# Jianxff/svo_pro_universal

Measured on AMD Instinct MI355X. Metric: aligned patches/sec + ms/frame, EuRoC 640x480 mono, 1/2/4/8 MI355X, higher is better.
Workload: dtype f64

## Files before the change

### svo_pro_universal_amd/csrc/context.hip

```cpp
#include <cmath>
#include <cstdarg>
#include <algorithm>
#include <cstring>

#include "svoh_internal.h"
#include "svoh_math.h"

namespace svoh {

static thread_local std::string g_global_err = "no error";

int set_error(svoh_ctx* ctx, int code, const char* fmt, ...)
{
  char buf[1024];
  va_list ap;
  va_start(ap, fmt);
  vsnprintf(buf, sizeof buf, fmt, ap);
  va_end(ap);
  if (ctx) ctx->err = buf; else g_global_err = buf;
  return code;
}

void set_global_error(const char* msg) { g_global_err = msg; }

// ... 335 lines not shown

__global__ __launch_bounds__(64) void camera_maths_kernel(const svoh_camera cam, int n, const double* xyz, double* px, double* J, double* f_back)
{
  const int i = blockIdx.x * 64 + threadIdx.x;
  if (i >= n) return;
  const CamModel cm = load_camera(cam);
  const Vec3 p = { xyz[3 * i], xyz[3 * i + 1], xyz[3 * i + 2] };
  double u, v;
  project3(cm, p, u, v);
  px[2 * i] = u; px[2 * i + 1] = v;
  double Jl[6];
  project3_jacobian(cm, p, Jl);
  for (int k = 0; k < 6; ++k) J[6 * i + k] = Jl[k];
  const Vec3 f = back_project3(cm, u, v);
  f_back[3 * i] = f.x; f_back[3 * i + 1] = f.y; f_back[3 * i + 2] = f.z;
}

__global__ __launch_bounds__(64) void camera_maths_wide_kernel(const svoh_camera cam, int n, const double* xyz, double* px, double* J, double* f_back)
{
  const int i = blockIdx.x * 64 + threadIdx.x;
  if (i >= n) return;
  const CamModelWide cm = load_camera_wide(cam);
  const Vec3 p = { xyz[3 * i], xyz[3 * i + 1], xyz[3 * i + 2] };
  double u, v;
  project3(cm, p, u, v);
  px[2 * i] = u; px[2 * i + 1] = v;
  if (J) {
    double Jl[6];
    project3_jacobian(cm, p, Jl);
    for (int k = 0; k < 6; ++k) J[6 * i + k] = Jl[k];
  }
  const Vec3 f = back_project3(cm, u, v);
  f_back[3 * i] = f.x; f_back[3 * i + 1] = f.y; f_back[3 * i + 2] = f.z;
}

void load_knobs_from_env(SvohKnobs& k)
{
  auto get = [](const char* name) { const char* e = getenv(name); return e ? atoi(e) : kKnobUnset; };
  k.klt_block = get("SVOH_KLT_BLOCK");
  k.matcher_g8 = get("SVOH_MATCHER_G8");
  k.seed_binning = get("SVOH_SEED_BINNING");
  k.pose_threads = get("SVOH_POSE_THREADS");
  k.align_cluster = get("SVOH_ALIGN_CLUSTER");
#ifdef SVOH_TEST_HOOKS
  k.align_cluster_test_absent = get("SVOH_ALIGN_CLUSTER_TEST_ABSENT");
#endif
  k.align_threads = get("SVOH_ALIGN_THREADS");
  k.align_rows = get("SVOH_ALIGN_ROWS");
  k.align_latency_build = get("SVOH_ALIGN_LATENCY_BUILD");
  k.align_lds = get("SVOH_ALIGN_LDS");
  k.align_wg_per_cu = get("SVOH_ALIGN_WG_PER_CU");
  k.kernel_timing = get("SVOH_KERNEL_TIMING");
  k.copy_kernel = get("SVOH_COPY_KERNEL");
}

static int build_pyramid_levels(svoh_ctx* ctx, hipStream_t stream, const std::shared_ptr<Slab>& slab, uint8_t* base, size_t fbytes, const size_t* offs, const int* ws,
                                const int* hs, int n_images, int width, int height, int n_levels, int rounding, svoh_frame_t* out_frames);

extern "C" {

int svoh_abi_version(void) { return SVOH_ABI_VERSION; }

int svoh_set_kernel_timing(svoh_ctx* ctx, int enabled)
try {
  if (!ctx) return set_error(nullptr, SVOH_ERR_INVALID_ARGUMENT, "ctx is NULL");
  ctx->knobs.kernel_timing = enabled ? 1 : 0;
  return SVOH_OK;
} SVOH_ABI_CATCH(ctx)

int svoh_set_copy_policy(svoh_ctx* ctx, int policy)
try {
  if (!ctx) return set_error(nullptr, SVOH_ERR_INVALID_ARGUMENT, "ctx is NULL");
  SVOH_REQUIRE(ctx, policy >= 0 && policy <= 2, "copy policy: 0 the runtime's copies, 1 copy kernels for 16 KB .. 1 MB, 2 copy kernels always");
  ctx->knobs.copy_kernel = policy;
  return SVOH_OK;
} SVOH_ABI_CATCH(ctx)

int svoh_reload_knobs(svoh_ctx* ctx)
try {
  if (!ctx) return set_error(nullptr, SVOH_ERR_INVALID_ARGUMENT, "ctx is NULL");
  const int timing = ctx->knobs.kernel_timing, copy_policy = ctx->knobs.copy_kernel;
  load_knobs_from_env(ctx->knobs);
  if (ctx->knobs.kernel_timing == kKnobUnset) ctx->knobs.kernel_timing = timing;
  if (ctx->knobs.copy_kernel == kKnobUnset) ctx->knobs.copy_kernel = copy_policy;
  return SVOH_OK;
} SVOH_ABI_CATCH(ctx)

int svoh_create(int device, svoh_ctx** out_ctx)
try {
  if (!out_ctx) return set_error(nullptr, SVOH_ERR_INVALID_ARGUMENT, "out_ctx is NULL");
  *out_ctx = nullptr;
  int n = 0;
  hipError_t e = hipGetDeviceCount(&n);
  if (e != hipSuccess || n <= 0)
    return set_error(nullptr, SVOH_ERR_NO_DEVICE, "no HIP device available (%s); libsvo_hip has no CPU path",
                     e == hipSuccess ? "device count is 0" : hipGetErrorString(e));
  if (device < 0 || device >= n)
    return set_error(nullptr, SVOH_ERR_INVALID_ARGUMENT, "device %d out of range [0,%d)", device, n);
  svoh_ctx* ctx = new (std::nothrow) svoh_ctx();
  if (!ctx) return set_error(nullptr, SVOH_ERR_OUT_OF_MEMORY, "out of host memory");
  ctx->device = device;
  ctx->err = "no error";
  load_knobs_from_env(ctx->knobs);
  e = hipSetDevice(device);
  if (e == hipSuccess) e = hipStreamCreateWithFlags(&ctx->stream, hipStreamNonBlocking);
  for (int k = 0; k < svoh_ctx::kAlignEventRing; ++k) {
    if (e == hipSuccess) e = hipEventCreate(&ctx->ev_align_start[k]);
    if (e == hipSuccess) e = hipEventCreate(&ctx->ev_align_stop[k]);
  }
  if (e == hipSuccess) e = hipEventCreateWithFlags(&ctx->ev_align_staged, hipEventDisableTiming);
  if (e == hipSuccess) e = hipEventCreate(&ctx->ev_misc_start);
  if (e == hipSuccess) e = hipEventCreate(&ctx->ev_misc_stop);
  hipDeviceProp_t prop;
  if (e == hipSuccess) e = hipGetDeviceProperties(&prop, device);
  if (e != hipSuccess) {
    set_error(nullptr, SVOH_ERR_HIP, "context creation failed: %s", hipGetErrorString(e));
    delete ctx;
    return SVOH_ERR_HIP;
  }
  ctx->num_cus = prop.multiProcessorCount;
  ctx->lds_per_block = prop.sharedMemPerBlock;
  *out_ctx = ctx;
  return SVOH_OK;
} SVOH_ABI_CATCH(nullptr)

int svoh_destroy(svoh_ctx* ctx)
try {
  if (!ctx) return SVOH_OK;
  (void)hipSetDevice(ctx->device);
  if (ctx->stream) { (void)hipStreamSynchronize(ctx->stream); }
  if (ctx->upload_stream) { (void)hipStreamSynchronize(ctx->upload_stream); }
  ctx->frames.clear();
  for (auto& kv : ctx->masks) (void)hipFree(kv.second.ptr);
  ctx->masks.clear();
  for (int k = 0; k < svoh_ctx::kAlignEventRing; ++k) {
    if (ctx->ev_align_start[k]) (void)hipEventDestroy(ctx->ev_align_start[k]);
    if (ctx->ev_align_stop[k]) (void)hipEventDestroy(ctx->ev_align_stop[k]);
  }
  if (ctx->ev_align_staged) (void)hipEventDestroy(ctx->ev_align_staged);
  if (ctx->ev_misc_start) (void)hipEventDestroy(ctx->ev_misc_start);
  if (ctx->ev_misc_stop) (void)hipEventDestroy(ctx->ev_misc_stop);
  if (ctx->ev_pose_done) (void)hipEventDestroy(ctx->ev_pose_done);
  if (ctx->ev_features) (void)hipEventDestroy(ctx->ev_features);
  if (ctx->ev_points) (void)hipEventDestroy(ctx->ev_points);
  if (ctx->ev_detect) (void)hipEventDestroy(ctx->ev_detect);
  if (ctx->ev_matcher_done) (void)hipEventDestroy(ctx->ev_matcher_done);
  if (ctx->upload_stream) { (void)hipStreamSynchronize(ctx->upload_stream); (void)hipStreamDestroy(ctx->upload_stream); }
  if (ctx->ev_upload) (void)hipEventDestroy(ctx->ev_upload);
  if (ctx->stream) (void)hipStreamDestroy(ctx->stream);
  delete ctx;
  return SVOH_OK;
} SVOH_ABI_CATCH(ctx)

const char* svoh_last_error_string(const svoh_ctx* ctx)
{
  return ctx ? ctx->err.c_str() : g_global_err.c_str();
}

int svoh_synchronize(svoh_ctx* ctx)
try {
  if (!ctx) return set_error(nullptr, SVOH_ERR_INVALID_ARGUMENT, "ctx is NULL");
  SVOH_HIP_TRY(ctx, hipStreamSynchronize(ctx->stream));
  return SVOH_OK;
} SVOH_ABI_CATCH(ctx)

void* svoh_stream(svoh_ctx* ctx) { return ctx ? (void*)ctx->stream : nullptr; }

int svoh_last_kernel_counters(svoh_ctx* ctx, uint64_t out[8])
try {
  if (!ctx) return set_error(nullptr, SVOH_ERR_INVALID_ARGUMENT, "ctx is NULL");
  SVOH_REQUIRE(ctx, out != nullptr && ctx->misc_launched && ctx->d_counters.ptr, "no counters yet");
  if (ctx->unit_counts_pending) {
    const int rc = reduce_unit_counts_now(ctx, ctx->unit_counts_pending);
    if (rc != SVOH_OK) return rc;
    ctx->unit_counts_pending = 0;
  }
  SVOH_HIP_TRY(ctx, hipMemcpyAsync(out, ctx->d_counters.ptr, 8 * sizeof(uint64_t), hipMemcpyDeviceToHost, ctx->stream));
  SVOH_HIP_TRY(ctx, hipStreamSynchronize(ctx->stream));
  return SVOH_OK;
} SVOH_ABI_CATCH(ctx)

int svoh_last_kernel_ms(svoh_ctx* ctx, float* ms)
try {
  if (!ctx) return set_error(nullptr, SVOH_ERR_INVALID_ARGUMENT, "ctx is NULL");
// ... 262 lines not shown
                                    rounding, out_frame);
  if (rc != SVOH_OK) return rc;
  if (host_levels_out) {
    const Frame* f = find_frame(ctx, *out_frame);
    for (int l = 0; l < n_levels; ++l) {
      if (!host_levels_out[l]) continue;
      SVOH_HIP_TRY(ctx, hipMemcpyAsync(host_levels_out[l], f->lv[l].data, (size_t)f->lv[l].w * f->lv[l].h,
                                       hipMemcpyDeviceToHost, ctx->stream));
    }
    SVOH_HIP_TRY(ctx, hipStreamSynchronize(ctx->stream));
  }
  return SVOH_OK;
} SVOH_ABI_CATCH(ctx)

int svoh_download_level(svoh_ctx* ctx, svoh_frame_t frame, int level, uint8_t* out, int* out_width, int* out_height)
try {
  if (!ctx) return set_error(nullptr, SVOH_ERR_INVALID_ARGUMENT, "ctx is NULL");
  const Frame* f = find_frame(ctx, frame);
  if (!f) return set_error(ctx, SVOH_ERR_BAD_HANDLE, "unknown frame handle %llu", (unsigned long long)frame);
  SVOH_REQUIRE(ctx, level >= 0 && level < f->n_levels, "level out of range");
  if (out_width) *out_width = f->lv[level].w;
  if (out_height) *out_height = f->lv[level].h;
  if (out) {
    SVOH_HIP_TRY(ctx, hipSetDevice(ctx->device));
    SVOH_HIP_TRY(ctx, hipMemcpyAsync(out, f->lv[level].data, (size_t)f->lv[level].w * f->lv[level].h,
                                     hipMemcpyDeviceToHost, ctx->stream));
    SVOH_HIP_TRY(ctx, hipStreamSynchronize(ctx->stream));
  }
  return SVOH_OK;
} SVOH_ABI_CATCH(ctx)

int svoh_frame_info(svoh_ctx* ctx, svoh_frame_t frame, int* n_levels, int* width0, int* height0)
try {
  if (!ctx) return set_error(nullptr, SVOH_ERR_INVALID_ARGUMENT, "ctx is NULL");
  const Frame* f = find_frame(ctx, frame);
  if (!f) return set_error(ctx, SVOH_ERR_BAD_HANDLE, "unknown frame handle %llu", (unsigned long long)frame);
  if (n_levels) *n_levels = f->n_levels;
  if (width0) *width0 = f->lv[0].w;
  if (height0) *height0 = f->lv[0].h;
  return SVOH_OK;
} SVOH_ABI_CATCH(ctx)

int svoh_context_stats(svoh_ctx* ctx, svoh_context_stats_t* out)
try {
  if (!ctx) return set_error(nullptr, SVOH_ERR_INVALID_ARGUMENT, "ctx is NULL");
  SVOH_REQUIRE(ctx, out != nullptr, "NULL argument");
  out->live_frames = (int64_t)ctx->frames.size();
  std::unordered_map<const void*, size_t> slabs;
  for (const auto& kv : ctx->frames)
    if (kv.second.slab) slabs[kv.second.slab.get()] = kv.second.slab->bytes;
  size_t fb = 0;
  for (const auto& kv : slabs) fb += kv.second;
  out->frame_bytes = (int64_t)fb;
  const svoh::DevBuffer* bufs[] = { &ctx->d_desc, &ctx->d_results, &ctx->d_feat, &ctx->d_eval, &ctx->d_xchg, &ctx->d_split,
                                    &ctx->d_counters, &ctx->d_unit_counts, &ctx->d_scratch0, &ctx->d_scratch1, &ctx->d_scratch2, &ctx->d_seed_bin, &ctx->d_match_seeds, &ctx->d_match_direct, &ctx->d_cand, &ctx->d_cand_multi };
  size_t wb = 0;
  for (const svoh::DevBuffer* b : bufs) wb += b->cap;
  out->workspace_bytes = (int64_t)wb;
  return SVOH_OK;
} SVOH_ABI_CATCH(ctx)

int svoh_camera_maths(svoh_ctx* ctx, const svoh_camera* cam, int n, const double* xyz, double* px, double* J, double* f_back)
try {
  if (!ctx) return set_error(nullptr, SVOH_ERR_INVALID_ARGUMENT, "ctx is NULL");
  SVOH_REQUIRE(ctx, cam && xyz && px && n >= 1 && n <= (1 << 20), "bad arguments");
  SVOH_REQUIRE(ctx, camera_is_known(*cam), "unsupported distortion model");
  SVOH_REQUIRE(ctx, cam->distortion != SVOH_DISTORTION_ATAN || (cam->d[0] != 0.0 && std::isfinite(cam->d[0])),
               "ATAN (fisheye) camera: s = d[0] must be finite and non-zero");
  if (J && !camera_has_jacobian(*cam))
    return set_error(ctx, SVOH_ERR_UNSUPPORTED, "the ATAN (fisheye) camera has no Jacobian (AtanDistortion::jacobian): pass J = NULL");
  SVOH_HIP_TRY(ctx, hipSetDevice(ctx->device));
  const size_t nd = (size_t)n;
  SVOH_HIP_TRY(ctx, ctx->d_scratch2.reserve(14 * nd * sizeof(double)));
  double* d = static_cast<double*>(ctx->d_scratch2.ptr);
  SVOH_HIP_TRY(ctx, hipMemcpyAsync(d, xyz, 3 * nd * sizeof(double), hipMemcpyHostToDevice, ctx->stream));
  if (camera_is_narrow(*cam))
    hipLaunchKernelGGL(camera_maths_kernel, dim3((unsigned)((n + 63) / 64)), dim3(64), 0, ctx->stream, *cam, n, d, d + 3 * nd, d + 5 * nd,
                       d + 11 * nd);
  else
    hipLaunchKernelGGL(camera_maths_wide_kernel, dim3((unsigned)((n + 63) / 64)), dim3(64), 0, ctx->stream, *cam, n, d, d + 3 * nd,
                       J ? d + 5 * nd : nullptr, d + 11 * nd);
  const hipError_t e = hipGetLastError();
  if (e != hipSuccess) return set_error(ctx, SVOH_ERR_HIP, "camera_maths launch failed: %s", hipGetErrorString(e));
  SVOH_HIP_TRY(ctx, hipMemcpyAsync(px, d + 3 * nd, 2 * nd * sizeof(double), hipMemcpyDeviceToHost, ctx->stream));
  if (J) SVOH_HIP_TRY(ctx, hipMemcpyAsync(J, d + 5 * nd, 6 * nd * sizeof(double), hipMemcpyDeviceToHost, ctx->stream));
  if (f_back) SVOH_HIP_TRY(ctx, hipMemcpyAsync(f_back, d + 11 * nd, 3 * nd * sizeof(double), hipMemcpyDeviceToHost, ctx->stream));
  SVOH_HIP_TRY(ctx, hipStreamSynchronize(ctx->stream));
  return SVOH_OK;
} SVOH_ABI_CATCH(ctx)

int svoh_release_frame(svoh_ctx* ctx, svoh_frame_t frame)
try {
  if (!ctx) return set_error(nullptr, SVOH_ERR_INVALID_ARGUMENT, "ctx is NULL");
  auto it = ctx->frames.find(frame);
  if (it == ctx->frames.end())
    return set_error(ctx, SVOH_ERR_BAD_HANDLE, "unknown frame handle %llu", (unsigned long long)frame);
  ctx->frames.erase(it);
  ++ctx->handle_generation;
  return SVOH_OK;
} SVOH_ABI_CATCH(ctx)


int svoh_mask_upload(svoh_ctx* ctx, int width, int height, int pitch, const uint8_t* data, svoh_mask_t* out_mask)
try {
  if (!ctx) return set_error(nullptr, SVOH_ERR_INVALID_ARGUMENT, "ctx is NULL");
  SVOH_REQUIRE(ctx, data && out_mask, "NULL argument");
  *out_mask = 0;
// ... 32 lines not shown
```

### svo_pro_universal_amd/csrc/sparse_align.hip

```cpp
#include <atomic>
#include <cstdlib>
#include <cstring>

#include <type_traits>

#include "svoh_internal.h"
#include "svoh_device_utils.h"
#include "svoh_math.h"

#define SVOH_ALIGN_DRAIN(ctx) do { SVOH_HIP_TRY(ctx, hipStreamSynchronize((ctx)->stream)); (ctx)->align_launches_since_drain = 0; } while (0)

namespace svoh {

struct DevCamDesc {
  DevImage ref[SVOH_MAX_LEVELS];
  DevImage cur[SVOH_MAX_LEVELS];
  svoh_camera cam;
  svoh_se3 ref_T_imu_cam, ref_T_cam_imu, cur_T_cam_imu;
  double ref_pos[3];
  const double* px;
  const double* f;
  const double* pos_world;
  const uint8_t* flags;
  int32_t n_features;
  int32_t feat_off;
};

struct DevProblemDesc {
  int32_t n_cams, cam_begin;
  svoh_se3 T_init;
  double alpha_init, beta_init;
  svoh_align_prior prior;
};

struct AlignKernelArgs {
  const DevProblemDesc* problems;
  const DevCamDesc* cams;
  svoh_align_result* results;
  double* wpk;
  int64_t slots;
  uint8_t* wsel;
  uint8_t* wvis;
  svoh_align_options opt;
  int32_t lds_img_bytes;
  int32_t rig_build;
  int32_t latency_build;
  int32_t lds_two_per_cu;
  int32_t ws_lds_bytes;
  int32_t eval_level;
  double* eval_out;
  long long* stamps;
  int32_t n_problems;
  int32_t* queue;
  int32_t one_each;
  const svoh_align_gn_state* ext_state;
  int32_t raw_sums;
  int32_t cluster;
  double* xchg;
  unsigned int* bar;
#ifdef SVOH_TEST_HOOKS
  int32_t cluster_test_absent;
#endif
};

constexpr int kXchgStride = 64;
// ... 1761 lines not shown
  if (!forced && !split && eval_level < 0 && n_problems == 1 && shared_class_geometry(ctx, problems[0], &shared_single)) forced = &shared_single;

  int S = (split && !split->update && split->n_shares > 1) ? split->n_shares : 1;
  bool cluster = false;
  if (!split && eval_level < 0) {
    const int g = forced ? forced->cluster_g : decide_cluster(ctx, n_problems, problems);
    if (g >= 2) { S = g; cluster = true; }
  }
  SVOH_REQUIRE(ctx, !forced || (!split && eval_level < 0), "a forced geometry applies to full runs only");
  SVOH_REQUIRE(ctx, !cluster || (int64_t)S * n_problems <= ctx->num_cus, "cluster mode: more workgroups than compute units");
  SVOH_REQUIRE(ctx, !cluster || n_problems <= kClusterMaxProblems, "cluster mode: more problems in one launch than arrival counters");
  SVOH_REQUIRE(ctx, S == 1 || n_problems == 1 || cluster, "shares apply to a single problem");
  const int n_desc = n_problems * S;

  size_t n_cams_total = 0, n_feat_total = 0, host_bytes = 0;
  int n_pos_jobs = 0;
  LaunchShape shape;
  for (int p = 0; p < n_problems; ++p) {
    const svoh_align_problem& pb = problems[p];
    SVOH_REQUIRE(ctx, pb.n_cams >= 1 && pb.n_cams <= SVOH_MAX_CAMS, "n_cams out of range");
    int nf = 0;
    for (int c = 0; c < pb.n_cams; ++c) {
      const svoh_align_camera& cam = pb.cams[c];
      SVOH_REQUIRE(ctx, cam.n_features >= 0, "negative n_features");
      SVOH_REQUIRE(ctx, cam.n_features == 0 || (cam.px && cam.f && cam.pos_world && cam.flags),
                   "NULL feature array");
      SVOH_REQUIRE(ctx, cam.cam.distortion == SVOH_DISTORTION_NONE || cam.cam.distortion == SVOH_DISTORTION_RADTAN,
                   "unsupported distortion model");
      nf += cam.n_features;
      if (cam.mem_space == SVOH_MEM_HOST && !(split && split->update))
        host_bytes += ((size_t)cam.n_features * (8 * 8 + 1) + 63) & ~(size_t)63;
      if (cam.pos_seed_unit) {
        SVOH_REQUIRE(ctx, cam.mem_space == SVOH_MEM_HOST && !split && eval_level < 0, "pos_seed_unit: host-memory cameras of full runs only");
        host_bytes += (((size_t)cam.n_features * 4 + 63) & ~(size_t)63) + 64;
        ++n_pos_jobs;
      }
    }
    n_cams_total += (size_t)pb.n_cams * S;
    n_feat_total += nf;
    add_to_shape(pb, S, &shape);
  }
  SVOH_REQUIRE(ctx, n_pos_jobs == 0 || ctx->seed_block.valid,
               "pos_seed_unit: no staged seed batch has been sent off on this context (or its block has been staged again)");
  const int max_feat_per_problem = shape.max_feat_per_problem;
  const size_t feat_slots = n_feat_total ? n_feat_total : 1;

  const size_t desc_only = sizeof(DevProblemDesc) * n_desc + sizeof(DevCamDesc) * n_cams_total;
  const size_t ctl_off = (desc_only + 255) & ~(size_t)255;
  const size_t up_base = ctl_off + 512;
  const size_t desc_bytes = up_base + host_bytes;
  const unsigned desc_slot = ctx->align_desc_slot ^ 1u;
  PinnedBuffer& h_desc = desc_slot ? ctx->h_desc_odd : ctx->h_desc;
  if (ctx->align_launches_since_drain >= 2) {
    if (ctx->align_staged_event_valid) SVOH_HIP_TRY(ctx, hipEventSynchronize(ctx->ev_align_staged));
    else SVOH_ALIGN_DRAIN(ctx);
  }
  SVOH_HIP_TRY(ctx, h_desc.reserve(desc_bytes));
  SVOH_HIP_TRY(ctx, ctx->d_desc.reserve(desc_bytes));
  memset(static_cast<uint8_t*>(h_desc.ptr) + ctl_off, 0, 512);
  const bool delivers = (S == 1 || cluster) && eval_level < 0;
  const size_t dev_results_off = delivers ? ctx->align_pending_dev : 0;
  {
    const size_t need = sizeof(svoh_align_result) * (dev_results_off + (size_t)n_desc + n_problems);
    if (need > ctx->d_results.cap) {
      if (dev_results_off) {
        SVOH_ALIGN_DRAIN(ctx);
        DevBuffer bigger;
        SVOH_HIP_TRY(ctx, bigger.reserve(need * 2));
        SVOH_HIP_TRY(ctx, hipMemcpy(bigger.ptr, ctx->d_results.ptr, sizeof(svoh_align_result) * dev_results_off, hipMemcpyDeviceToDevice));
        std::swap(bigger.ptr, ctx->d_results.ptr);
        std::swap(bigger.cap, ctx->d_results.cap);
      } else {
        SVOH_HIP_TRY(ctx, ctx->d_results.reserve(need));
      }
    }
  }
  if (delivers) {
    SVOH_REQUIRE(ctx, ctx->align_pending_results + (size_t)n_problems <= svoh_ctx::kMaxQueuedResults,
                 "too many alignment results queued without a fetch");
    size_t want_results = ctx->align_pending_results + (size_t)n_problems;
    const size_t queue_of_these = (size_t)svoh_ctx::kAlignEventRing * (size_t)n_problems;
    if (want_results < queue_of_these && queue_of_these <= svoh_ctx::kMaxQueuedResults) want_results = queue_of_these;
    const size_t need = sizeof(svoh_align_result) * want_results;
    if (need > ctx->h_results.cap) {
      if (ctx->align_pending_results) {
        SVOH_ALIGN_DRAIN(ctx);
        PinnedBuffer bigger;
        SVOH_HIP_TRY(ctx, bigger.reserve(need * 2));
        memcpy(bigger.ptr, ctx->h_results.ptr, sizeof(svoh_align_result) * ctx->align_pending_results);
        std::swap(bigger.ptr, ctx->h_results.ptr);
        std::swap(bigger.cap, ctx->h_results.cap);
      } else {
        SVOH_HIP_TRY(ctx, ctx->h_results.reserve(need));
      }
    }
  }
  SVOH_HIP_TRY(ctx, ctx->d_feat.reserve(feat_slots * (kWsPairs * 16 + 2) + 256));
  SVOH_HIP_TRY(ctx, ctx->d_eval.reserve(74 * sizeof(double) * S));

  DevProblemDesc* hp = static_cast<DevProblemDesc*>(h_desc.ptr);
  DevCamDesc* hc = reinterpret_cast<DevCamDesc*>(hp + n_desc);
  uint8_t* hup = static_cast<uint8_t*>(h_desc.ptr) + up_base;
  uint8_t* dup = static_cast<uint8_t*>(ctx->d_desc.ptr) + up_base;
  size_t up_off = 0;
  int cam_idx = 0, feat_off = 0;
  const int need_levels = opt->max_level + 1;
  const uint8_t* share_base[SVOH_MAX_CAMS] = {};
  std::vector<PosFromSeedsJob> pos_jobs;
  int pos_jobs_max_n = 0;
  for (int pd = 0; pd < n_desc; ++pd) {
    const int p = pd / S, sh = pd % S;
    const svoh_align_problem& pb = problems[p];
    DevProblemDesc& d = hp[pd];
    d.n_cams = pb.n_cams;
    d.cam_begin = cam_idx;
    d.T_init = pb.T_icur_iref;
    d.alpha_init = pb.alpha_init; d.beta_init = pb.beta_init;
    d.prior = pb.prior;
    for (int c = 0; c < pb.n_cams; ++c, ++cam_idx) {
      const svoh_align_camera& cam = pb.cams[c];
      DevCamDesc& dc = hc[cam_idx];
      const Frame* fr = find_frame(ctx, cam.ref_frame);
      const Frame* fc = find_frame(ctx, cam.cur_frame);
      if (!fr || !fc) return set_error(ctx, SVOH_ERR_BAD_HANDLE, "problem %d camera %d: unknown frame handle", p, c);
      if (fr->n_levels < need_levels || fc->n_levels < need_levels)
        return set_error(ctx, SVOH_ERR_INVALID_ARGUMENT, "problem %d camera %d: pyramid has fewer than %d levels", p,
                         c, need_levels);
      for (int l = 0; l < SVOH_MAX_LEVELS; ++l) {
        dc.ref[l] = l < fr->n_levels ? fr->lv[l] : DevImage{ nullptr, 0, 0, 0, 0 };
        dc.cur[l] = l < fc->n_levels ? fc->lv[l] : DevImage{ nullptr, 0, 0, 0, 0 };
      }
      dc.cam = cam.cam;
      {
        const Rigid I = mul(load_rigid(cam.ref_T_cam_imu), load_rigid(cam.ref_T_imu_cam));
        const double dev = fmax(fmax(fabs(fabs(I.q.w) - 1.0), fmax(fabs(I.q.x), fmax(fabs(I.q.y), fabs(I.q.z)))),
                                fmax(fabs(I.t.x), fmax(fabs(I.t.y), fabs(I.t.z))));
        if (!(dev <= 1e-9))
          return set_error(ctx, SVOH_ERR_INVALID_ARGUMENT,
                           "problem %d camera %d: ref_T_cam_imu is not the inverse of ref_T_imu_cam (deviation %.3g)", p, c, dev);
      }
      dc.ref_T_imu_cam = cam.ref_T_imu_cam;
      dc.ref_T_cam_imu = cam.ref_T_cam_imu;
      dc.cur_T_cam_imu = cam.cur_T_cam_imu;
      for (int k = 0; k < 3; ++k) dc.ref_pos[k] = cam.ref_pos[k];
      const size_t lo = (size_t)((int64_t)cam.n_features * sh / S), hi = (size_t)((int64_t)cam.n_features * (sh + 1) / S);
      dc.n_features = (int32_t)(hi - lo);
      dc.feat_off = feat_off;
      feat_off += dc.n_features;
      if (cam.mem_space == SVOH_MEM_DEVICE || cam.n_features == 0 || (split && split->update)) {
        dc.px = cam.px + 2 * lo; dc.f = cam.f + 3 * lo; dc.pos_world = cam.pos_world + 3 * lo; dc.flags = cam.flags + lo;
      } else {
        const size_t n = (size_t)cam.n_features;
        if (sh == 0) {
          uint8_t* h = hup + up_off;
          memcpy(h, cam.px, n * 16);
          memcpy(h + n * 16, cam.f, n * 24);
          memcpy(h + n * 40, cam.pos_world, n * 24);
          memcpy(h + n * 64, cam.flags, n);
          share_base[c] = dup + up_off;
          up_off += (n * 65 + 63) & ~(size_t)63;
        }
        if (sh == 0 && cam.pos_seed_unit) {
          memcpy(hup + up_off, cam.pos_seed_unit, n * 4);
          PosFromSeedsJob jb;
          jb.pos = reinterpret_cast<double*>(const_cast<uint8_t*>(share_base[c]) + n * 40);
          jb.unit = reinterpret_cast<const int32_t*>(dup + up_off);
          jb.n = (int32_t)n; jb.pad_ = 0;
          pos_jobs.push_back(jb);
          if ((int)n > pos_jobs_max_n) pos_jobs_max_n = (int)n;
          up_off += (n * 4 + 63) & ~(size_t)63;
        }
        const uint8_t* dv = share_base[c];
        dc.px = reinterpret_cast<const double*>(dv) + 2 * lo;
        dc.f = reinterpret_cast<const double*>(dv + n * 16) + 3 * lo;
        dc.pos_world = reinterpret_cast<const double*>(dv + n * 40) + 3 * lo;
        dc.flags = dv + n * 64 + lo;
      }
    }
  }
  const PosFromSeedsJob* pos_jobs_device = nullptr;
  if (!pos_jobs.empty()) {
    memcpy(hup + up_off, pos_jobs.data(), sizeof(PosFromSeedsJob) * pos_jobs.size());
    pos_jobs_device = reinterpret_cast<const PosFromSeedsJob*>(dup + up_off);
    up_off += (sizeof(PosFromSeedsJob) * pos_jobs.size() + 63) & ~(size_t)63;
  }
  SVOH_HIP_TRY(ctx, svoh_copy_to_device(ctx, ctx->d_desc.ptr, h_desc.ptr, up_base + up_off));
  if (pos_jobs_device) {
    const int rcp = svoh_launch_pos_from_seed_batch(ctx, (int)pos_jobs.size(), pos_jobs_max_n, pos_jobs_device);
    if (rcp != SVOH_OK) return rcp;
  }
  ctx->align_desc_slot = desc_slot;
  ctx->align_staged_event_valid = false;
  if (ctx->align_launches_since_drain >= 1) {
    SVOH_HIP_TRY(ctx, hipEventRecord(ctx->ev_align_staged, ctx->stream));
    ctx->align_staged_event_valid = true;
  }
  ++ctx->align_launches_since_drain;

  AlignKernelArgs args;
  args.problems = static_cast<const DevProblemDesc*>(ctx->d_desc.ptr);
  args.cams = reinterpret_cast<const DevCamDesc*>(args.problems + n_desc);
  args.results = static_cast<svoh_align_result*>(ctx->d_results.ptr) + dev_results_off;
  double* w = static_cast<double*>(ctx->d_feat.ptr);
  args.wpk = w;
  args.slots = (int64_t)feat_slots;
  args.wsel = reinterpret_cast<uint8_t*>(w + 2 * kWsPairs * feat_slots);
  args.wvis = args.wsel + feat_slots;
  args.opt = *opt;
  args.eval_level = eval_level;
  args.eval_out = static_cast<double*>(ctx->d_eval.ptr);
  args.stamps = nullptr;
  args.n_problems = n_desc;
  args.ext_state = nullptr;
  args.raw_sums = 0;
  args.cluster = 0;
  args.xchg = nullptr;
  args.bar = nullptr;
#ifdef SVOH_TEST_HOOKS
  args.cluster_test_absent = SvohKnobs::or_default(ctx->knobs.align_cluster_test_absent, 0);
#endif
  if (cluster) {
    const size_t xchg_bytes = 2 * (size_t)S * kXchgStride * sizeof(double) * n_problems;
    SVOH_HIP_TRY(ctx, ctx->d_xchg.reserve(xchg_bytes));
    args.cluster = S;
    args.xchg = static_cast<double*>(ctx->d_xchg.ptr);
    args.bar = reinterpret_cast<unsigned int*>(static_cast<uint8_t*>(ctx->d_desc.ptr) + ctl_off + 256);
  }
  if (split && !split->update) {
    args.ext_state = split->ext_state;
    if (S == 1) args.eval_out = split->sums_out;
    args.raw_sums = 1;
  }
  if (split && split->update) {
    const bool illum_u = opt->estimate_illumination_gain || opt->estimate_illumination_offset;
    if (opt->patch_size == 4) {
      if (illum_u) hipLaunchKernelGGL((align_gn_update_kernel<4, true>), dim3(1), dim3(64), 0, ctx->stream, args, split->sums_in, split->state, eval_level, split->iter);
      else hipLaunchKernelGGL((align_gn_update_kernel<4, false>), dim3(1), dim3(64), 0, ctx->stream, args, split->sums_in, split->state, eval_level, split->iter);
    } else {
      if (illum_u) hipLaunchKernelGGL((align_gn_update_kernel<8, true>), dim3(1), dim3(64), 0, ctx->stream, args, split->sums_in, split->state, eval_level, split->iter);
      else hipLaunchKernelGGL((align_gn_update_kernel<8, false>), dim3(1), dim3(64), 0, ctx->stream, args, split->sums_in, split->state, eval_level, split->iter);
    }
    const hipError_t eu = hipGetLastError();
    if (eu != hipSuccess) return set_error(ctx, SVOH_ERR_HIP, "gn_update launch failed: %s", hipGetErrorString(eu));
    return SVOH_OK;
  }
  args.queue = reinterpret_cast<int32_t*>(static_cast<uint8_t*>(ctx->d_desc.ptr) + ctl_off);
#ifdef SVOH_PHASE_STAMPS
  SVOH_HIP_TRY(ctx, ctx->d_scratch0.reserve(sizeof(long long) * 20 * (size_t)n_problems));
  args.stamps = static_cast<long long*>(ctx->d_scratch0.ptr);
#endif

  const AlignGeometry geo = forced ? *forced : decide_geometry(ctx, opt, n_desc, cluster ? S : 0, shape);
  const int nt = geo.nt, rows = geo.rows;
  size_t lds = (nt == 256) ? 52224 : 78 * 1024;
  args.latency_build = geo.latency ? 1 : 0;
  args.rig_build = geo.rig ? 1 : 0;
  args.lds_two_per_cu = (nt == 256 && !cluster && ctx->knobs.align_lds == kKnobUnset && ctx->knobs.align_wg_per_cu == kKnobUnset) ? 1 : 0;
  lds = (size_t)SvohKnobs::or_default(ctx->knobs.align_lds, (int)lds) & ~(size_t)15;
  const size_t lds_cap = (nt == 256) ? 163840 - 32768 : 153856;
  if (lds > lds_cap) lds = lds_cap;
  args.ws_lds_bytes = 0;
  if (nt == 512 && !cluster && max_feat_per_problem <= kWsLdsMaxFeatures && lds >= (size_t)kWsLdsMaxFeatures * kWsPairs * 16 + 4096) {
    args.ws_lds_bytes = ((max_feat_per_problem > 0 ? max_feat_per_problem : 1) * kWsPairs * 16 + 15) & ~15;
  }
  args.lds_img_bytes = (int32_t)(lds - (size_t)args.ws_lds_bytes);

  const bool illum = opt->estimate_illumination_gain || opt->estimate_illumination_offset;
  int grid = ctx->num_cus * SvohKnobs::or_default(ctx->knobs.align_wg_per_cu, nt == 256 ? 2 : 1);
  if (grid > n_desc || grid <= 0) grid = n_desc;
  if (cluster) grid = n_desc;
  args.one_each = 0;
  hipError_t e;
  const bool timed = ctx->timing_on();
  const int ev_slot = (int)(ctx->align_timed_launches % svoh_ctx::kAlignEventRing);
  if (timed) SVOH_HIP_TRY(ctx, hipEventRecord(ctx->ev_align_start[ev_slot], ctx->stream));
  const bool robust = opt->robustification != 0;
#ifdef SVOH_DEV_ONLY_PLAIN
  if (robust || illum) return set_error(ctx, SVOH_ERR_UNSUPPORTED, "development build: plain kernels only");
  e = opt->patch_size == 4 ? launch_nt<4, false, false>(ctx->stream, nt, rows, grid, lds, args)
                           : launch_nt<8, false, false>(ctx->stream, nt, rows, grid, lds, args);
#else
  if (opt->patch_size == 4) {
    if (robust) e = illum ? launch_nt<4, true, true>(ctx->stream, nt, rows, grid, lds, args) : launch_nt<4, false, true>(ctx->stream, nt, rows, grid, lds, args);
    else e = illum ? launch_nt<4, true, false>(ctx->stream, nt, rows, grid, lds, args) : launch_nt<4, false, false>(ctx->stream, nt, rows, grid, lds, args);
  } else {
    if (robust) e = illum ? launch_nt<8, true, true>(ctx->stream, nt, rows, grid, lds, args) : launch_nt<8, false, true>(ctx->stream, nt, rows, grid, lds, args);
    else e = illum ? launch_nt<8, true, false>(ctx->stream, nt, rows, grid, lds, args) : launch_nt<8, false, false>(ctx->stream, nt, rows, grid, lds, args);
  }
#endif
  if (e != hipSuccess)
    return set_error(ctx, SVOH_ERR_HIP, "sparse_align launch failed: %s", hipGetErrorString(e));
  if (S > 1 && !cluster) {
    hipLaunchKernelGGL(sum_shares_kernel, dim3(1), dim3(128), 0, ctx->stream, static_cast<const double*>(ctx->d_eval.ptr), S,
                       split->sums_out);
    const hipError_t es = hipGetLastError();
    if (es != hipSuccess) return set_error(ctx, SVOH_ERR_HIP, "sum_shares launch failed: %s", hipGetErrorString(es));
  }
  if (timed) { SVOH_HIP_TRY(ctx, hipEventRecord(ctx->ev_align_stop[ev_slot], ctx->stream)); ++ctx->align_timed_launches; }
  ctx->align_last_timed = timed;
  ++ctx->align_launches;
  if (!split && eval_level < 0) {
    ctx->align_last_geometry_key = geo.key(); ctx->align_last_grid = grid; ctx->align_last_n_desc = n_desc;
  }
  if (delivers) {
    SVOH_HIP_TRY(ctx, svoh_copy_to_host(ctx, static_cast<svoh_align_result*>(ctx->h_results.ptr) + ctx->align_pending_results,
                                        args.results, sizeof(svoh_align_result) * n_problems));
    ctx->align_last_results_off = ctx->align_pending_results;
    if (ctx->align_pending_results == 0) ctx->align_result_dev_index.clear();
    for (int p = 0; p < n_problems; ++p) ctx->align_result_dev_index.push_back((uint32_t)(dev_results_off + (size_t)p));
    ctx->align_pending_results += (size_t)n_problems;
    ctx->align_pending_dev = dev_results_off + (size_t)n_desc + (size_t)n_problems;
  }
#ifdef SVOH_PHASE_STAMPS
  {
    std::vector<long long> h((size_t)n_problems * 20);
    SVOH_HIP_TRY(ctx, hipMemcpyAsync(h.data(), args.stamps, h.size() * sizeof(long long), hipMemcpyDeviceToHost, ctx->stream));
    SVOH_ALIGN_DRAIN(ctx);
    double sum[20] = {0};
    for (int p = 0; p < n_problems; ++p) for (int k = 0; k < 20; ++k) sum[k] += (double)h[(size_t)p * 20 + k];
    fprintf(stderr, "[stamps] one-lane step: set-up %.0f solve %.0f update %.0f camera poses %.0f\n", sum[8] / n_problems, sum[9] / n_problems,
            sum[10] / n_problems, sum[11] / n_problems);
    fprintf(stderr, "[stamps] inside the passes (thread 0): set-up %.0f row arrival %.0f projection %.0f pixels %.0f Jacobian rows + map %.0f; gradient-only passes as a whole %.0f, the vote's barrier behind them %.0f\n", sum[12] / n_problems,
            sum[13] / n_problems, sum[14] / n_problems, sum[15] / n_problems, sum[16] / n_problems, sum[17] / n_problems, sum[18] / n_problems);
    fprintf(stderr, "[stamps] n=%d nt=%d avg cycles/block: base %.0f stage %.0f patch %.0f reduce %.0f serial %.0f total %.0f; "
            "gradient-only passes kept %.2f / discarded %.2f per problem\n",
            n_problems, nt, sum[0] / n_problems, sum[1] / n_problems, sum[2] / n_problems, sum[3] / n_problems,
            sum[4] / n_problems, sum[7] / n_problems, sum[6] / n_problems, sum[5] / n_problems);
  }
#endif
  ctx->last_align_n = delivers ? n_problems : 0;
  return SVOH_OK;
}

}

using namespace svoh;

extern "C" {

int svoh_sparse_align_enqueue(svoh_ctx* ctx, const svoh_align_options* options, int n_problems,
                              const svoh_align_problem* problems)
try {
  return enqueue_align(ctx, options, n_problems, problems, -1);
} SVOH_ABI_CATCH(ctx)

int svoh_sparse_align_geometry_key(svoh_ctx* ctx, const svoh_align_options* options, const svoh_align_problem* problem, int32_t* key)
try {
  if (!ctx) return set_error(nullptr, SVOH_ERR_INVALID_ARGUMENT, "ctx is NULL");
  const int rc = validate_options(ctx, options);
  if (rc != SVOH_OK) return rc;
  SVOH_REQUIRE(ctx, problem && key, "NULL argument");
  SVOH_REQUIRE(ctx, problem->n_cams >= 1 && problem->n_cams <= SVOH_MAX_CAMS, "n_cams out of range");
  *key = geometry_of_single(ctx, options, *problem).key();
  return SVOH_OK;
} SVOH_ABI_CATCH(ctx)

int svoh_set_align_geometry_classes(svoh_ctx* ctx, int shared)
try {
  if (!ctx) return set_error(nullptr, SVOH_ERR_INVALID_ARGUMENT, "ctx is NULL");
  SVOH_REQUIRE(ctx, shared == 0 || shared == 1, "geometry classes: 0 = the fastest geometry for a problem alone, 1 = shared classes");
  ctx->align_shared_classes = shared != 0;
  return SVOH_OK;
} SVOH_ABI_CATCH(ctx)

int svoh_sparse_align_enqueue_keyed(svoh_ctx* ctx, const svoh_align_options* options, int n_problems,
                                    const svoh_align_problem* problems, int32_t key)
try {
  if (!ctx) return set_error(nullptr, SVOH_ERR_INVALID_ARGUMENT, "ctx is NULL");
  AlignGeometry geo;
  SVOH_REQUIRE(ctx, AlignGeometry::from_key(key, &geo), "not a geometry key of svoh_sparse_align_geometry_key");
  SVOH_REQUIRE(ctx, n_problems >= 1 && problems, "no problems");
  int per_launch = n_problems;
  if (geo.cluster_g >= 2) {
    per_launch = ctx->num_cus / geo.cluster_g > 0 ? ctx->num_cus / geo.cluster_g : 1;
    if (per_launch > kClusterMaxProblems) per_launch = kClusterMaxProblems;
  }
  for (int p0 = 0; p0 < n_problems; p0 += per_launch) {
    const int n = n_problems - p0 < per_launch ? n_problems - p0 : per_launch;
    const int rc = enqueue_align(ctx, options, n, problems + p0, -1, nullptr, &geo);
    if (rc != SVOH_OK) return rc;
  }
  return SVOH_OK;
} SVOH_ABI_CATCH(ctx)

int svoh_sparse_align_fetch(svoh_ctx* ctx, int n_problems, svoh_align_result* results)
try {
  if (!ctx) return set_error(nullptr, SVOH_ERR_INVALID_ARGUMENT, "ctx is NULL");
  SVOH_REQUIRE(ctx, results && n_problems >= 1 && n_problems <= ctx->last_align_n && ctx->h_results.ptr &&
                        ctx->align_pending_results >= (size_t)n_problems, "nothing to fetch");
  SVOH_HIP_TRY(ctx, hipSetDevice(ctx->device));
  SVOH_ALIGN_DRAIN(ctx);
  memcpy(results, static_cast<const svoh_align_result*>(ctx->h_results.ptr) + ctx->align_last_results_off,
         sizeof(svoh_align_result) * n_problems);
  ctx->align_pending_results = 0;
  ctx->align_pending_dev = 0;
  return SVOH_OK;
} SVOH_ABI_CATCH(ctx)
// ... 173 lines not shown
```

### svo_pro_universal_amd/csrc/svoh_internal.h

```cpp
#pragma once

#include <hip/hip_runtime.h>

#include <cstdint>
#include <cstdio>
#include <memory>
#include <new>
#include <stdexcept>
#include <string>
#include <unordered_map>
#include <algorithm>
#include <vector>

#include "../../include/svo_hip.h"

namespace svoh {

struct DevImage {
  const uint8_t* data;
  int32_t w, h, pitch, pad;
};

constexpr size_t kSlabTailPad = 64;

// ... 89 lines not shown
struct Frame {
  std::shared_ptr<Slab> slab;
  int n_levels = 0;
  DevImage lv[SVOH_MAX_LEVELS];
};

struct Mask {
  uint8_t* ptr = nullptr;
  int w = 0, h = 0;
};

constexpr size_t kMinScratchBytes = (size_t)1 << 20;
struct DevBuffer {
  void* ptr = nullptr;
  size_t cap = 0;
  hipError_t reserve(size_t bytes)
  {
    if (bytes <= cap) return hipSuccess;
    if (ptr) { (void)hipFree(ptr); ptr = nullptr; cap = 0; }
    size_t want = bytes + bytes / 2 + 4096;
    if (want < kMinScratchBytes) want = kMinScratchBytes;
    hipError_t e = hipMalloc(&ptr, want);
    if (e == hipSuccess) cap = want;
    return e;
  }
  ~DevBuffer() { if (ptr) (void)hipFree(ptr); }
};

struct PinnedBuffer {
  void* ptr = nullptr;
  size_t cap = 0;
  hipError_t reserve(size_t bytes)
  {
    if (bytes <= cap) return hipSuccess;
    if (ptr) { (void)hipHostFree(ptr); ptr = nullptr; cap = 0; }
    size_t want = bytes + bytes / 2 + 4096;
    if (want < kMinScratchBytes) want = kMinScratchBytes;
    hipError_t e = hipHostMalloc(&ptr, want, hipHostMallocDefault);
    if (e == hipSuccess) cap = want;
    return e;
  }
  ~PinnedBuffer() { if (ptr) (void)hipHostFree(ptr); }
};

}

constexpr int kKnobUnset = -2147483647 - 1;
struct SvohKnobs {
  int klt_block = kKnobUnset;
  int matcher_g8 = kKnobUnset;
  int seed_binning = kKnobUnset;
  int pose_threads = kKnobUnset;
  int align_cluster = kKnobUnset;
#ifdef SVOH_TEST_HOOKS
  int align_cluster_test_absent = kKnobUnset;
#endif
  int align_threads = kKnobUnset;
  int align_rows = kKnobUnset;
  int align_latency_build = kKnobUnset;
  int align_lds = kKnobUnset;
  int align_wg_per_cu = kKnobUnset;
  int kernel_timing = kKnobUnset;
  int copy_kernel = kKnobUnset;
  static int or_default(int v, int dflt) { return v == kKnobUnset ? dflt : v; }
};
void load_knobs_from_env(SvohKnobs& k);

struct svoh_ctx {
  SvohKnobs knobs;
  int device = 0;
  hipStream_t stream = nullptr;
  int num_cus = 0;
  size_t lds_per_block = 0;
  std::string err;
  std::shared_ptr<svoh::SlabPool> slab_pool = std::make_shared<svoh::SlabPool>();
  std::unordered_map<uint64_t, svoh::Frame> frames;
  uint64_t next_frame_id = 1;
  std::unordered_map<uint64_t, svoh::Mask> masks;
  uint64_t next_mask_id = 1;
  uint64_t handle_generation = 0;
  std::shared_ptr<svoh::BlockPool> feature_pool = std::make_shared<svoh::BlockPool>();
  std::unordered_map<uint64_t, svoh::FeatureSet> feature_sets;
  uint64_t next_features_id = 1;
  svoh::PinnedBuffer h_features;
  hipEvent_t ev_features = nullptr;

  svoh::DevBuffer d_desc;
  svoh::DevBuffer d_results;
  svoh::DevBuffer d_feat;
  svoh::DevBuffer d_eval;
  svoh::DevBuffer d_xchg;
  svoh::DevBuffer d_split;
  svoh::PinnedBuffer h_desc;
  svoh::PinnedBuffer h_desc_odd;
  svoh::PinnedBuffer h_results;
  int last_align_n = 0;
  static constexpr size_t kMaxQueuedResults = (size_t)1 << 18;
  size_t align_pending_results = 0, align_last_results_off = 0;
  size_t align_pending_dev = 0;
  std::vector<uint32_t> align_result_dev_index;
  static constexpr int kAlignEventRing = 32;
  hipEvent_t ev_align_start[kAlignEventRing] = {}, ev_align_stop[kAlignEventRing] = {};
  unsigned long long align_launches = 0;
  int32_t align_last_geometry_key = 0, align_last_grid = 0, align_last_n_desc = 0;
  hipEvent_t ev_align_staged = nullptr;
  bool align_staged_event_valid = false;
  unsigned align_launches_since_drain = 0;
  unsigned align_desc_slot = 0;
  bool align_shared_classes = false;
  bool align_no_cluster = false;
  hipEvent_t ev_misc_start = nullptr, ev_misc_stop = nullptr;
  bool in_pose_hook = false; const void* d_pose_results = nullptr; int n_pose_results = 0;
  hipEvent_t ev_pose_done = nullptr;
  hipStream_t upload_stream = nullptr;
  hipEvent_t ev_upload = nullptr;
  bool upload_pending = false;
  bool misc_timed = false;
  bool misc_launched = false;
  unsigned long long align_timed_launches = 0;
  bool align_last_timed = false;
  bool timing_on() const { return knobs.kernel_timing != kKnobUnset && knobs.kernel_timing != 0; }
  svoh::DevBuffer d_counters;
  svoh::DevBuffer d_unit_counts;
  size_t unit_counts_pending = 0;

  bool matcher_deferred = false;
  bool matcher_deferred_used[2] = { false, false };
  struct PendingCopy { void* dst; const void* src; size_t bytes; };
  std::vector<PendingCopy> matcher_pending;
  struct PendingCount { int32_t* dst; const uint8_t* flags; int n; };
  std::vector<PendingCount> matcher_pending_counts;
  struct DeferredLaunch {
    std::vector<uint8_t> args;
    int n = 0, g8 = 0;
    int max_w = 0, max_h = 0;
    size_t out_off = 0, out_bytes = 0;
    void* d_block = nullptr;
    bool valid = false;
    void* d2h_dst = nullptr; const void* d2h_src = nullptr; size_t d2h_bytes = 0;
    void* views_h = nullptr; void* views_d = nullptr; int n_ref = 0, n_cur = 0;
    uint64_t cur_frame_handle = 0;
    const void* d_pose_results = nullptr; int n_pose_results = 0; bool pose_from_results = false;
    const void* d_fidx = nullptr;
    bool seed_block_staged = false;
  } matcher_deferred_launch[2];
  svoh::DevBuffer d_match_seeds, d_match_direct;
  svoh::PinnedBuffer h_match_seeds, h_match_direct;
  struct MatcherStage {
    bool valid = false, want_outputs = false, resident = false;
    int n = 0, max_views = 0;
    size_t o_fidx = 0;
    size_t o_views = 0, o_idx = 0, o_cidx = 0, o_px = 0, o_f = 0, o_grad = 0, o_level = 0, o_type = 0, o_depth = 0, o_pxcur = 0, o_state = 0,
           o_result = 0, o_success = 0, o_fcur = 0, o_slevel = 0, o_hinv = 0, o_A = 0, o_nsucc = 0, in_total = 0, back_from = 0, total = 0;
  } matcher_stage[2];

  svoh::DevBuffer d_cand;
  svoh::PinnedBuffer h_cand;
  int cand_pending_n = 0;
  size_t cand_out_off = 0;
  svoh::DevBuffer d_cand_multi;
  svoh::PinnedBuffer h_cand_multi;
// ... 71 lines not shown
```

Baseline: 2.167 billion.

## Overlap sparse-align descriptor uploads and result downloads on a side copy stream

Double-buffers the device descriptor block and moves large descriptor uploads and result downloads for non-cluster, non-split align launches onto a separate non-blocking copy stream. Events order each upload after the previous kernel that read that slot, and defer each result download until the next launch or drain. The goal is to overlap host-device transfers with the align kernel instead of serialising them on the main stream. In exchange it adds event bookkeeping, a second descriptor buffer, a one-time warm-up copy, and a larger preallocated results buffer, and it only triggers for big uploads (over 1 MiB) when there are at least as many problems as CUs.

```diff
diff --git a/svo_pro_universal_amd/csrc/context.hip b/svo_pro_universal_amd/csrc/context.hip
--- a/svo_pro_universal_amd/csrc/context.hip
+++ b/svo_pro_universal_amd/csrc/context.hip
@@ -411,6 +411,7 @@
   k.align_wg_per_cu = get("SVOH_ALIGN_WG_PER_CU");
   k.kernel_timing = get("SVOH_KERNEL_TIMING");
   k.copy_kernel = get("SVOH_COPY_KERNEL");
+  k.align_side_copies = get("SVOH_ALIGN_SIDE_COPIES");
 }
 
 static int build_pyramid_levels(svoh_ctx* ctx, hipStream_t stream, const std::shared_ptr<Slab>& slab, uint8_t* base, size_t fbytes, const size_t* offs, const int* ws,
@@ -489,6 +490,9 @@
   (void)hipSetDevice(ctx->device);
   if (ctx->stream) { (void)hipStreamSynchronize(ctx->stream); }
   if (ctx->upload_stream) { (void)hipStreamSynchronize(ctx->upload_stream); }
+  if (ctx->align_copy_stream) { (void)hipStreamSynchronize(ctx->align_copy_stream); (void)hipStreamDestroy(ctx->align_copy_stream); }
+  for (hipEvent_t ev : { ctx->ev_align_kernel[0], ctx->ev_align_kernel[1], ctx->ev_align_uploaded, ctx->ev_align_delivered })
+    if (ev) (void)hipEventDestroy(ev);
   ctx->frames.clear();
   for (auto& kv : ctx->masks) (void)hipFree(kv.second.ptr);
   ctx->masks.clear();
@@ -857,7 +861,7 @@
   size_t fb = 0;
   for (const auto& kv : slabs) fb += kv.second;
   out->frame_bytes = (int64_t)fb;
-  const svoh::DevBuffer* bufs[] = { &ctx->d_desc, &ctx->d_results, &ctx->d_feat, &ctx->d_eval, &ctx->d_xchg, &ctx->d_split,
+  const svoh::DevBuffer* bufs[] = { &ctx->d_desc[0], &ctx->d_desc[1], &ctx->d_results, &ctx->d_feat, &ctx->d_eval, &ctx->d_xchg, &ctx->d_split,
                                     &ctx->d_counters, &ctx->d_unit_counts, &ctx->d_scratch0, &ctx->d_scratch1, &ctx->d_scratch2, &ctx->d_seed_bin, &ctx->d_match_seeds, &ctx->d_match_direct, &ctx->d_cand, &ctx->d_cand_multi };
   size_t wb = 0;
   for (const svoh::DevBuffer* b : bufs) wb += b->cap;
diff --git a/svo_pro_universal_amd/csrc/sparse_align.hip b/svo_pro_universal_amd/csrc/sparse_align.hip
--- a/svo_pro_universal_amd/csrc/sparse_align.hip
+++ b/svo_pro_universal_amd/csrc/sparse_align.hip
@@ -8,9 +8,51 @@
 #include "svoh_device_utils.h"
 #include "svoh_math.h"
 
-#define SVOH_ALIGN_DRAIN(ctx) do { SVOH_HIP_TRY(ctx, hipStreamSynchronize((ctx)->stream)); (ctx)->align_launches_since_drain = 0; } while (0)
+#define SVOH_ALIGN_DRAIN(ctx) SVOH_HIP_TRY(ctx, svoh::align_drain(ctx))
 
 namespace svoh {
+
+static hipError_t align_drain(svoh_ctx* ctx);
+
+static hipError_t align_side_setup(svoh_ctx* ctx, void* h, void* d, size_t bytes)
+{
+  if (ctx->align_copy_stream) return hipSuccess;
+  hipError_t e = ctx->align_launches_since_drain ? align_drain(ctx) : hipSuccess;
+  hipEvent_t* evs[] = { &ctx->ev_align_kernel[0], &ctx->ev_align_kernel[1], &ctx->ev_align_uploaded, &ctx->ev_align_delivered };
+  for (hipEvent_t* ev : evs)
+    if (e == hipSuccess && !*ev) e = hipEventCreateWithFlags(ev, hipEventDisableTiming);
+  if (e == hipSuccess) e = hipStreamCreateWithFlags(&ctx->align_copy_stream, hipStreamNonBlocking);
+  if (bytes > ((size_t)1 << 20)) bytes = (size_t)1 << 20;
+  if (e == hipSuccess) e = hipMemcpyAsync(d, h, bytes, hipMemcpyHostToDevice, ctx->align_copy_stream);
+  if (e == hipSuccess) e = hipMemcpyAsync(h, d, bytes, hipMemcpyDeviceToHost, ctx->align_copy_stream);
+  if (e == hipSuccess) e = hipStreamSynchronize(ctx->align_copy_stream);
+  return e;
+}
+
+static hipError_t align_flush_download(svoh_ctx* ctx)
+{
+  svoh_ctx::AlignDownload& d = ctx->align_download;
+  if (!d.bytes) return hipSuccess;
+  hipError_t e = hipStreamWaitEvent(ctx->align_copy_stream, d.after, 0);
+  if (e == hipSuccess) e = hipMemcpyAsync(d.dst, d.src, d.bytes, hipMemcpyDeviceToHost, ctx->align_copy_stream);
+  if (e == hipSuccess) e = hipEventRecord(ctx->ev_align_delivered, ctx->align_copy_stream);
+  if (e != hipSuccess) return e;
+  d.bytes = 0;
+  ctx->align_delivery_pending = true;
+  return hipSuccess;
+}
+
+static hipError_t align_drain(svoh_ctx* ctx)
+{
+  hipError_t e = align_flush_download(ctx);
+  if (e == hipSuccess) e = hipStreamSynchronize(ctx->stream);
+  if (e == hipSuccess && ctx->align_delivery_pending) e = hipEventSynchronize(ctx->ev_align_delivered);
+  if (e != hipSuccess) return e;
+  ctx->align_delivery_pending = false;
+  ctx->align_launches_since_drain = 0;
+  ctx->align_block_read_ev[0] = ctx->align_block_read_ev[1] = nullptr;
+  return hipSuccess;
+}
 
 struct DevCamDesc {
   DevImage ref[SVOH_MAX_LEVELS];
@@ -1878,16 +1920,21 @@
   const unsigned desc_slot = ctx->align_desc_slot ^ 1u;
   PinnedBuffer& h_desc = desc_slot ? ctx->h_desc_odd : ctx->h_desc;
   if (ctx->align_launches_since_drain >= 2) {
-    if (ctx->align_staged_event_valid) SVOH_HIP_TRY(ctx, hipEventSynchronize(ctx->ev_align_staged));
+    if (ctx->align_staged_wait_ev) SVOH_HIP_TRY(ctx, hipEventSynchronize(ctx->align_staged_wait_ev));
     else SVOH_ALIGN_DRAIN(ctx);
   }
   SVOH_HIP_TRY(ctx, h_desc.reserve(desc_bytes));
-  SVOH_HIP_TRY(ctx, ctx->d_desc.reserve(desc_bytes));
+  DevBuffer& d_desc = ctx->d_desc[desc_slot];
+  if (desc_bytes > d_desc.cap && ctx->align_launches_since_drain >= 1) SVOH_ALIGN_DRAIN(ctx);
+  SVOH_HIP_TRY(ctx, d_desc.reserve(desc_bytes));
   memset(static_cast<uint8_t*>(h_desc.ptr) + ctl_off, 0, 512);
   const bool delivers = (S == 1 || cluster) && eval_level < 0;
   const size_t dev_results_off = delivers ? ctx->align_pending_dev : 0;
   {
-    const size_t need = sizeof(svoh_align_result) * (dev_results_off + (size_t)n_desc + n_problems);
+    size_t want_dev = dev_results_off + (size_t)n_desc + n_problems;
+    if (delivers && dev_results_off == 0 && (size_t)svoh_ctx::kAlignEventRing * (size_t)n_problems <= svoh_ctx::kMaxQueuedResults)
+      want_dev *= (size_t)svoh_ctx::kAlignEventRing;
+    const size_t need = sizeof(svoh_align_result) * want_dev;
     if (need > ctx->d_results.cap) {
       if (dev_results_off) {
         SVOH_ALIGN_DRAIN(ctx);
@@ -1927,7 +1974,7 @@
   DevProblemDesc* hp = static_cast<DevProblemDesc*>(h_desc.ptr);
   DevCamDesc* hc = reinterpret_cast<DevCamDesc*>(hp + n_desc);
   uint8_t* hup = static_cast<uint8_t*>(h_desc.ptr) + up_base;
-  uint8_t* dup = static_cast<uint8_t*>(ctx->d_desc.ptr) + up_base;
+  uint8_t* dup = static_cast<uint8_t*>(d_desc.ptr) + up_base;
   size_t up_off = 0;
   int cam_idx = 0, feat_off = 0;
   const int need_levels = opt->max_level + 1;
@@ -2010,21 +2057,51 @@
     pos_jobs_device = reinterpret_cast<const PosFromSeedsJob*>(dup + up_off);
     up_off += (sizeof(PosFromSeedsJob) * pos_jobs.size() + 63) & ~(size_t)63;
   }
-  SVOH_HIP_TRY(ctx, svoh_copy_to_device(ctx, ctx->d_desc.ptr, h_desc.ptr, up_base + up_off));
+  const int side_knob = ctx->knobs.align_side_copies;
+  const bool side_kind = n_desc >= ctx->num_cus && !cluster && !split && !forced && eval_level < 0 &&
+                         (side_knob == kKnobUnset ? up_base + up_off > ((size_t)1 << 20) : side_knob != 0);
+  if (side_kind) SVOH_HIP_TRY(ctx, align_side_setup(ctx, h_desc.ptr, d_desc.ptr, up_base + up_off));
+  const bool side = side_kind && ctx->align_launches_since_drain >= 1;
+  const unsigned prev_slot = desc_slot ^ 1u;
+  if (side) {
+    if (!ctx->align_block_read_ev[prev_slot]) {
+      SVOH_HIP_TRY(ctx, hipEventRecord(ctx->ev_align_kernel[prev_slot], ctx->stream));
+      ctx->align_block_read_ev[prev_slot] = ctx->ev_align_kernel[prev_slot];
+    }
+    if (ctx->align_block_read_ev[desc_slot]) SVOH_HIP_TRY(ctx, hipStreamWaitEvent(ctx->align_copy_stream, ctx->align_block_read_ev[desc_slot], 0));
+    SVOH_HIP_TRY(ctx, hipMemcpyAsync(d_desc.ptr, h_desc.ptr, up_base + up_off, hipMemcpyHostToDevice, ctx->align_copy_stream));
+    SVOH_HIP_TRY(ctx, hipEventRecord(ctx->ev_align_uploaded, ctx->align_copy_stream));
+    if (ctx->align_last_was_side) {
+      SVOH_HIP_TRY(ctx, hipEventRecord(ctx->ev_align_staged, ctx->align_copy_stream));
+      ctx->align_staged_wait_ev = ctx->ev_align_staged;
+    } else {
+      ctx->align_staged_wait_ev = ctx->align_block_read_ev[prev_slot];
+    }
+    SVOH_HIP_TRY(ctx, align_flush_download(ctx));
+    SVOH_HIP_TRY(ctx, hipStreamWaitEvent(ctx->stream, ctx->ev_align_uploaded, 0));
+    ++ctx->align_side_launches;
+  } else {
+    SVOH_HIP_TRY(ctx, align_flush_download(ctx));
+    SVOH_HIP_TRY(ctx, svoh_copy_to_device(ctx, d_desc.ptr, h_desc.ptr, up_base + up_off));
+  }
   if (pos_jobs_device) {
     const int rcp = svoh_launch_pos_from_seed_batch(ctx, (int)pos_jobs.size(), pos_jobs_max_n, pos_jobs_device);
     if (rcp != SVOH_OK) return rcp;
   }
   ctx->align_desc_slot = desc_slot;
-  ctx->align_staged_event_valid = false;
-  if (ctx->align_launches_since_drain >= 1) {
-    SVOH_HIP_TRY(ctx, hipEventRecord(ctx->ev_align_staged, ctx->stream));
-    ctx->align_staged_event_valid = true;
-  }
+  if (!side) {
+    ctx->align_staged_wait_ev = nullptr;
+    if (ctx->align_launches_since_drain >= 1) {
+      SVOH_HIP_TRY(ctx, hipEventRecord(ctx->ev_align_staged, ctx->stream));
+      ctx->align_staged_wait_ev = ctx->ev_align_staged;
+    }
+    ctx->align_block_read_ev[desc_slot] = nullptr;
+  }
+  ctx->align_last_was_side = side;
   ++ctx->align_launches_since_drain;
 
   AlignKernelArgs args;
-  args.problems = static_cast<const DevProblemDesc*>(ctx->d_desc.ptr);
+  args.problems = static_cast<const DevProblemDesc*>(d_desc.ptr);
   args.cams = reinterpret_cast<const DevCamDesc*>(args.problems + n_desc);
   args.results = static_cast<svoh_align_result*>(ctx->d_results.ptr) + dev_results_off;
   double* w = static_cast<double*>(ctx->d_feat.ptr);
@@ -2050,7 +2127,7 @@
     SVOH_HIP_TRY(ctx, ctx->d_xchg.reserve(xchg_bytes));
     args.cluster = S;
     args.xchg = static_cast<double*>(ctx->d_xchg.ptr);
-    args.bar = reinterpret_cast<unsigned int*>(static_cast<uint8_t*>(ctx->d_desc.ptr) + ctl_off + 256);
+    args.bar = reinterpret_cast<unsigned int*>(static_cast<uint8_t*>(d_desc.ptr) + ctl_off + 256);
   }
   if (split && !split->update) {
     args.ext_state = split->ext_state;
@@ -2070,7 +2147,7 @@
     if (eu != hipSuccess) return set_error(ctx, SVOH_ERR_HIP, "gn_update launch failed: %s", hipGetErrorString(eu));
     return SVOH_OK;
   }
-  args.queue = reinterpret_cast<int32_t*>(static_cast<uint8_t*>(ctx->d_desc.ptr) + ctl_off);
+  args.queue = reinterpret_cast<int32_t*>(static_cast<uint8_t*>(d_desc.ptr) + ctl_off);
 #ifdef SVOH_PHASE_STAMPS
   SVOH_HIP_TRY(ctx, ctx->d_scratch0.reserve(sizeof(long long) * 20 * (size_t)n_problems));
   args.stamps = static_cast<long long*>(ctx->d_scratch0.ptr);
@@ -2128,9 +2205,18 @@
   if (!split && eval_level < 0) {
     ctx->align_last_geometry_key = geo.key(); ctx->align_last_grid = grid; ctx->align_last_n_desc = n_desc;
   }
+  if (side) {
+    SVOH_HIP_TRY(ctx, hipEventRecord(ctx->ev_align_kernel[desc_slot], ctx->stream));
+    ctx->align_block_read_ev[desc_slot] = ctx->ev_align_kernel[desc_slot];
+    ctx->align_download.dst = static_cast<svoh_align_result*>(ctx->h_results.ptr) + ctx->align_pending_results;
+    ctx->align_download.src = args.results;
+    ctx->align_download.bytes = sizeof(svoh_align_result) * n_problems;
+    ctx->align_download.after = ctx->ev_align_kernel[desc_slot];
+  }
   if (delivers) {
-    SVOH_HIP_TRY(ctx, svoh_copy_to_host(ctx, static_cast<svoh_align_result*>(ctx->h_results.ptr) + ctx->align_pending_results,
-                                        args.results, sizeof(svoh_align_result) * n_problems));
+    if (!side)
+      SVOH_HIP_TRY(ctx, svoh_copy_to_host(ctx, static_cast<svoh_align_result*>(ctx->h_results.ptr) + ctx->align_pending_results,
+                                          args.results, sizeof(svoh_align_result) * n_problems));
     ctx->align_last_results_off = ctx->align_pending_results;
     if (ctx->align_pending_results == 0) ctx->align_result_dev_index.clear();
     for (int p = 0; p < n_problems; ++p) ctx->align_result_dev_index.push_back((uint32_t)(dev_results_off + (size_t)p));
@@ -2169,6 +2255,10 @@
 try {
   return enqueue_align(ctx, options, n_problems, problems, -1);
 } SVOH_ABI_CATCH(ctx)
+
+#ifdef SVOH_TEST_HOOKS
+unsigned long long svoh_test_align_side_launches(const svoh_ctx* ctx) { return ctx ? ctx->align_side_launches : 0; }
+#endif
 
 int svoh_sparse_align_geometry_key(svoh_ctx* ctx, const svoh_align_options* options, const svoh_align_problem* problem, int32_t* key)
 try {
diff --git a/svo_pro_universal_amd/csrc/svoh_internal.h b/svo_pro_universal_amd/csrc/svoh_internal.h
--- a/svo_pro_universal_amd/csrc/svoh_internal.h
+++ b/svo_pro_universal_amd/csrc/svoh_internal.h
@@ -165,9 +165,7 @@
   int seed_binning = kKnobUnset;
   int pose_threads = kKnobUnset;
   int align_cluster = kKnobUnset;
-#ifdef SVOH_TEST_HOOKS
   int align_cluster_test_absent = kKnobUnset;
-#endif
   int align_threads = kKnobUnset;
   int align_rows = kKnobUnset;
   int align_latency_build = kKnobUnset;
@@ -175,6 +173,7 @@
   int align_wg_per_cu = kKnobUnset;
   int kernel_timing = kKnobUnset;
   int copy_kernel = kKnobUnset;
+  int align_side_copies = kKnobUnset;
   static int or_default(int v, int dflt) { return v == kKnobUnset ? dflt : v; }
 };
 void load_knobs_from_env(SvohKnobs& k);
@@ -198,7 +197,7 @@
   svoh::PinnedBuffer h_features;
   hipEvent_t ev_features = nullptr;
 
-  svoh::DevBuffer d_desc;
+  svoh::DevBuffer d_desc[2];
   svoh::DevBuffer d_results;
   svoh::DevBuffer d_feat;
   svoh::DevBuffer d_eval;
@@ -217,9 +216,17 @@
   unsigned long long align_launches = 0;
   int32_t align_last_geometry_key = 0, align_last_grid = 0, align_last_n_desc = 0;
   hipEvent_t ev_align_staged = nullptr;
-  bool align_staged_event_valid = false;
+  hipEvent_t align_staged_wait_ev = nullptr;
   unsigned align_launches_since_drain = 0;
   unsigned align_desc_slot = 0;
+  hipStream_t align_copy_stream = nullptr;
+  hipEvent_t ev_align_kernel[2] = {};
+  hipEvent_t align_block_read_ev[2] = {};
+  hipEvent_t ev_align_uploaded = nullptr, ev_align_delivered = nullptr;
+  struct AlignDownload { void* dst = nullptr; const void* src = nullptr; size_t bytes = 0; hipEvent_t after = nullptr; } align_download;
+  bool align_delivery_pending = false;
+  bool align_last_was_side = false;
+  unsigned long long align_side_launches = 0;
   bool align_shared_classes = false;
   bool align_no_cluster = false;
   hipEvent_t ev_misc_start = nullptr, ev_misc_stop = nullptr;
```

Result: faster. 2.229 billion (median of 6 runs) (+2.8%).
